# resero-labs/latok

Hardware: AMD Instinct MI355X
Metric: input UTF-8 GB/s tokenized (fused feature+split-mask path) (higher is better)
Workload: dtype u64

## Files before the change

### latok_amd/csrc/api.cpp

```cpp
#include <hip/hip_runtime.h>
#include <errno.h>
#include <fcntl.h>
#include <stdarg.h>
#include <stdio.h>
#include <stdlib.h>
#include <string.h>
#include <sys/mman.h>
#include <sys/stat.h>
#include <unistd.h>

#include <algorithm>
#include <array>
#include <atomic>
#include <chrono>
#include <mutex>
#include <new>
#include <string>
#include <thread>
#include <vector>

#include "../../include/latok_hip.h"
#include "corpus_gen.h"
#include "flow_hazards.h"
#include "kernels.h"
// ... 90 lines not shown
}
static bool wait_completion_word(const unsigned long long* word, unsigned long long seq) {
    const auto t0 = std::chrono::steady_clock::now();
    for (;;) {
        for (int i = 0; i < 256; ++i) {
            if (__atomic_load_n(word, __ATOMIC_ACQUIRE) == seq) return true;
            cpu_relax();
        }
        if (std::chrono::duration_cast<std::chrono::nanoseconds>(std::chrono::steady_clock::now() - t0).count() > kPollNs) return false;
    }
}

static inline size_t align16(size_t x) { return (x + 15) & ~(size_t)15; }

constexpr int64_t kSmallChars = 262144;
constexpr int64_t kSmallStrings = 16384;

enum class Form { Utf32, Latin1, Ucs2, Utf8 };
struct Input {
    const void* p = nullptr;
    Form form = Form::Utf32;
    size_t width() const { return form == Form::Utf32 ? 4 : form == Form::Ucs2 ? 2 : 1; }
    bool narrow() const { return form == Form::Latin1 || form == Form::Ucs2; }
};
static Form form_of_kind(int kind) { return kind == 4 ? Form::Utf32 : kind == 2 ? Form::Ucs2 : kind == 1 ? Form::Latin1 : Form::Utf8; }
struct Batch {
    Input in;
    const int64_t* row = nullptr;
    int64_t n_str = 0, total = 0;
};

struct Workspace {
    DevBuf summ, seg_agg, fix_count, tile_first;
    DevBuf bits, space, kept, wcnt, wpref, bases, scalar, chain, chain_ctl;
    DevBuf codes, widened;
    DevBuf lead, bspace, cpbits, cpspace, cprow;
    DevBuf jbody, jhead;
    unsigned scan_epoch = 0, chain_seen = 0, chain_ctl_seen = 0;
    bool chain_ready = false;
    void release() {
        for (DevBuf* b : {&summ, &seg_agg, &fix_count, &tile_first, &bits, &space, &kept, &wcnt, &wpref, &bases, &scalar, &chain,
                          &chain_ctl, &codes, &widened, &lead, &bspace, &cpbits, &cpspace, &cprow, &jbody, &jhead})
            b->release();
        scan_epoch = chain_seen = chain_ctl_seen = 0;
        chain_ready = false;
    }
};
struct WsNeed {
    DevBuf* buf;
    size_t bytes;
};
constexpr int kTileNeeds = 4;
constexpr int kWsNeeds = 22;
static std::array<WsNeed, kWsNeeds> ws_needs(Workspace& w, int64_t units, bool spans, bool feats, bool widen, int64_t cp_rows = 0,
                                             bool join = false) {
    const size_t t = (size_t)std::max<int64_t>((units + latok::kTile - 1) / latok::kTile, 1);
    const size_t words = (size_t)((units + 63) / 64), c_tiles = (words + 63) / 64;
    return {{{&w.summ, t * 16},
             {&w.seg_agg, (t / latok::kWPB + 2) * (sizeof(latok::Fn64) + sizeof(latok::Hd64))},
             {&w.fix_count, 8},
             {&w.tile_first, t * 8 + 8},
             {&w.bits, words * 8 + 8},
             {&w.space, spans ? words * 8 + 8 : 0},
             {&w.kept, spans ? words * 8 + 8 : 0},
             {&w.wcnt, c_tiles * 8 + 8},
             {&w.wpref, words * 2 + 8},
             {&w.bases, c_tiles * 8 + 8},
             {&w.scalar, 64},
             {&w.chain, (size_t)latok::count_blocks((int64_t)words) * 8 + 64},
             {&w.chain_ctl, 64},
             {&w.codes, feats ? (size_t)units + latok::kTile + 256 : 0},
             {&w.widened, widen ? (size_t)units * 4 + 16 : 0},
             {&w.lead, cp_rows > 0 ? words * 8 + 8 : 0},
             {&w.bspace, cp_rows > 0 && spans ? words * 8 + 8 : 0},
             {&w.cpbits, cp_rows > 0 ? words * 8 + 8 : 0},
             {&w.cpspace, cp_rows > 0 && spans ? words * 8 + 8 : 0},
             {&w.cprow, cp_rows > 0 ? (size_t)cp_rows * 8 : 0},
             {&w.jbody, join ? words * 8 + 8 : 0},
             {&w.jhead, join ? words * 8 + 8 : 0}}};
}
static int ws_ensure(const WsNeed* needs, int n) {
    for (int i = 0; i < n; ++i) {
        const int rc = needs[i].buf->ensure(needs[i].bytes);
        if (rc) return rc;
    }
    return LATOK_OK;
}

struct Ctx {
    std::mutex mu;
    bool inited = false;
    int device = -1, n_cu = 0;
    hipStream_t stream = nullptr;
    DevBuf t1, t1rule, t2code, t2cls, cw;
// ... 106 lines not shown
    hipEvent_t tiles_begin = nullptr, tiles_end = nullptr;
    hipStream_t st = nullptr;
};

int run_pipeline(Ctx& g, Workspace& w, const Pipe& a) {
    const int64_t n_str = a.b.n_str, total = a.b.total;
    if (total <= 0 || n_str <= 0) return LATOK_OK;
    const Input& in = a.b.in;
    int mode = a.mode;
    if (in.form != Form::Utf32) {
        if (mode != latok::kModeBits) return fail(LATOK_ERR_INVALID, "byte-space input supports the bitmask outputs only");
        if (((uintptr_t)in.p & 15) != 0)
            return fail(LATOK_ERR_INVALID, in.narrow() ? "device code-unit pointer must be 16-byte aligned" : "device UTF-8 pointer must be 16-byte aligned");
        mode = in.form == Form::Latin1 ? latok::kModeLatin1 : (in.form == Form::Ucs2 ? latok::kModeUcs2 : latok::kModeBytes);
    }
    if (g.rules_on && mode != latok::kModeBlockMask) mode = latok::mode_with_rules(mode);
    const int64_t n_tiles = (total + latok::kTile - 1) / latok::kTile;
    int rc = ws_ensure(ws_needs(w, total, false, false, false).data(), kTileNeeds);
    if (rc) return rc;
    latok::SplitParams P;
    P.cps = in.form == Form::Utf32 ? (const uint32_t*)in.p : nullptr;
    P.u8 = in.form == Form::Utf32 ? nullptr : (const uint8_t*)in.p;
    P.row_off = a.b.row;
    P.n_str = n_str;
    P.total = total;
    P.n_tiles = n_tiles;
    const int n_cu = g.plan_cus > 0 ? g.plan_cus : g.n_cu;
    const bool one_launch_ok = a.stages == 7 && in.form == Form::Utf32 && !a.tiles_begin && !a.tiles_end && one_segment_enabled();
    latok::LaunchPlan L;
    latok::plan_launch(n_tiles, n_cu, &w != &g.ws, mode, one_launch_ok, &L);
    P.seg_tiles = L.seg_tiles;
    P.n_segs = L.n_segs;
    const bool one_launch = L.one_launch != 0;
    if ((size_t)P.n_segs * (sizeof(latok::Fn64) + sizeof(latok::Hd64)) > w.seg_agg.cap || (size_t)n_tiles * 16 > w.summ.cap)
        return fail(LATOK_ERR_INVALID, "internal: workspace too small for %lld segments / %lld tiles", (long long)P.n_segs, (long long)n_tiles);
    if (a.codes && mode != latok::kModeBits && mode != latok::kModeRules)
        return fail(LATOK_ERR_INVALID, "internal: code bytes are written by the UTF-32 bitmask modes only");
    const uint8_t* tables = (const uint8_t*)((latok::mode_rules(mode) || a.codes) ? g.t1rule.p : g.t1.p);
    P.t1 = tables;
    P.t2 = tables + latok::kStage1Pad;
    if (latok::mode_base(mode) == latok::kModeBytes) {
        P.t1 = (const uint8_t*)(latok::mode_rules(mode) ? g.tb6rule.p : g.tb6.p);
        P.t2 = P.t1 + latok::kB6Stage1Bytes;
    }
    if (latok::mode_rules(mode)) P.rules = g.rules;
    else memset(&P.rules, 0, sizeof(P.rules));
    P.bits_out = a.bits;
    P.values_out = a.values;
    P.space_out = a.space;
    P.lead_out = a.lead;
    P.lead_pref_out = a.lead_pref;
    P.lead_cnt_out = a.lead_cnt;
    P.codes_out = a.codes;
    P.tile_first = (int64_t*)w.tile_first.p;
    P.summ = (int4*)w.summ.p;
    P.seg_fn = (latok::Fn64*)w.seg_agg.p;
    P.seg_hd = (latok::Hd64*)((char*)w.seg_agg.p + (size_t)P.n_segs * sizeof(latok::Fn64));
    P.fix_count = (int64_t*)w.fix_count.p;
    P.bm_a1 = a.bm_a1;
    P.bm_a2 = a.bm_a2;
    P.bm_flags = a.bm_flags;
    P.done = (a.stages & 4) ? a.done : latok::DoneSignal{nullptr, 0, nullptr};
    g.last.plan = L;
    g.last.n_tiles = n_tiles;
    g.last.mode = mode;
    g.last.small = g.pin.d && in.p == g.pin.d;
    g.last.fix_count = (const int64_t*)w.fix_count.p;
    g.last.st = a.st;
    g.last.valid = true;
    const hipStream_t st = a.st;
    if (one_launch) {
        HIP_TRY(latok::launch_one_segment(P, mode, st));
        return LATOK_OK;
    }
    if (a.stages & 1) HIP_TRY(latok::launch_tile_index(P, st));
    if (a.tiles_begin) HIP_TRY(hipEventRecord(a.tiles_begin, st));
    if (a.stages & 2) HIP_TRY(latok::launch_split_tiles(P, mode, L, st));
    if (a.tiles_end) HIP_TRY(hipEventRecord(a.tiles_end, st));
    if (a.stages & 4) HIP_TRY(latok::launch_resolve_fix(P, mode, L, st));
    return LATOK_OK;
}

int check_csr_host(const int64_t* row_off, int64_t n_str, int64_t* total_io) {
    if (n_str < 0) return fail(LATOK_ERR_INVALID, "n_str must be >= 0");
    if (n_str == 0) { *total_io = 0; return LATOK_OK; }
    if (!row_off) return fail(LATOK_ERR_INVALID, "row_off is NULL");
    if (row_off[0] != 0) return fail(LATOK_ERR_INVALID, "row_off[0] must be 0");
    for (int64_t s = 0; s < n_str; ++s)
        if (row_off[s + 1] < row_off[s]) return fail(LATOK_ERR_INVALID, "row_off must be non-decreasing");
    if (*total_io >= 0 && *total_io != row_off[n_str])
        return fail(LATOK_ERR_INVALID, "total_chars does not match row_off[n_str]");
    *total_io = row_off[n_str];
    return LATOK_OK;
}

int resolve_total_device(const int64_t* d_row, int64_t n_str, int64_t* total_io, hipStream_t st) {
    if (n_str < 0) return fail(LATOK_ERR_INVALID, "n_str must be >= 0");
    if (n_str == 0) { *total_io = 0; return LATOK_OK; }
    if (*total_io < 0) {
        HIP_TRY(hipMemcpyAsync(total_io, d_row + n_str, 8, hipMemcpyDeviceToHost, st));
        HIP_TRY(hipStreamSynchronize(st));
    }
    return LATOK_OK;
}

int resolve_total(const int64_t* row_off, int64_t n_str, int64_t* total_io, bool dev, hipStream_t st) {
    return dev ? resolve_total_device(row_off, n_str, total_io, st) : check_csr_host(row_off, n_str, total_io);
}

int arm_done(Ctx& g, hipStream_t st, latok::DoneSignal* done) {
    *done = latok::DoneSignal{nullptr, 0, nullptr};
    if (!poll_completion()) return LATOK_OK;
// ... 1815 lines not shown

int latok_debug_set_scan_epoch(unsigned epoch) {
    LATOK_ENTER();
    g.ws.scan_epoch = epoch & 0x3FFFFu;
    return LATOK_OK;
}

extern "C" int latok_debug_limits(int64_t* out, int n) {
    const int64_t v[15] = {latok::kTile, latok::kWPB, latok::kNarrowWPB, latok::kSegMax, latok::kOneSegTiles, latok::kFastTailTiles,
                           kSmallChars, kSmallStrings, latok::kCompressWaves, latok::kFeatWaves, latok::kFeatRound, latok::kFeatRoundTm,
                           latok::kFeatFormThresh, latok::kFeatWinBytes, latok::kHashWaveBytes};
    if (!out || n < 0) return fail(LATOK_ERR_INVALID, "NULL output");
    const int k = n < 15 ? n : 15;
    for (int i = 0; i < k; ++i) out[i] = v[i];
    return k;
}

static int put_plan(const latok::LaunchPlan& L, int64_t n_tiles, int64_t* out, int n) {
    const int64_t v[12] = {L.n_cu_eff, L.seg_tiles, L.n_segs, L.rounds, L.grid, L.one_launch ? 0 : L.grid, L.fast_tail, L.pf, L.wpb, L.nw,
                           L.one_launch, n_tiles};
    const int k = n < 12 ? n : 12;
    for (int i = 0; i < k; ++i) out[i] = v[i];
    return k;
}

extern "C" int latok_debug_plan(int64_t n_tiles, int n_cu, int in_flow, int mode, int64_t* out, int n) {
    if (!out || n < 0 || n_tiles < 1 || n_cu < 1 || mode < latok::kModeBits || mode > latok::kModeValuesRules)
        return fail(LATOK_ERR_INVALID, "n_tiles >= 1, n_cu >= 1, mode 0..%d", latok::kModeValuesRules);
    latok::LaunchPlan L;
    latok::plan_launch(n_tiles, n_cu, in_flow != 0, mode, one_segment_enabled(), &L);
    return put_plan(L, n_tiles, out, n);
}

extern "C" int latok_debug_set_plan_cus(int n_cu) {
    LATOK_ENTER();
    int rc = need_init(g);
    if (rc) return rc;
    if (n_cu != 0 && (n_cu < 8 || n_cu > g.n_cu)) return fail(LATOK_ERR_INVALID, "plan CUs must be 0 or 8..%d", g.n_cu);
    g.plan_cus = n_cu;
    return LATOK_OK;
}

extern "C" int latok_debug_last_plan(int64_t* out, int n) {
    LATOK_ENTER();
    int rc = need_init(g);
    if (rc) return rc;
    if (!out || n < 0) return fail(LATOK_ERR_INVALID, "NULL output");
    if (!g.last.valid) return 0;
    int64_t fix = 0;
    HIP_TRY(hipStreamSynchronize(g.last.st));
    HIP_TRY(hipMemcpy(&fix, g.last.fix_count, 8, hipMemcpyDeviceToHost));
    const int64_t head[3] = {g.last.mode, g.last.small ? 1 : 0, fix};
    int k = 0;
    for (; k < 3 && k < n; ++k) out[k] = head[k];
    if (n > 3) k += put_plan(g.last.plan, g.last.n_tiles, out + 3, n - 3);
    return k;
}

extern "C" int latok_debug_last_route(void) {
    LATOK_ENTER();
    return g.last_route;
}

extern "C" int latok_debug_flow_route(int n_slots, const uint64_t* lo, const uint64_t* bytes, const int* is_write, int n, int* drained_out) {
    static thread_local latok::FlowHazards held;
    static thread_local unsigned long long seq = 0;
// ... 939 lines not shown
```

### latok_amd/csrc/kernels.h

```cpp
#ifndef LATOK_KERNELS_H
#define LATOK_KERNELS_H
#include <hip/hip_runtime.h>
#include <stdint.h>

#include "split_code.h"

namespace latok {

constexpr int kTile = 4096;
constexpr int kTblShift = 7;
constexpr int kStage1Len = 8705;
constexpr int kStage1Pad = 8720;
constexpr int kStage2Len = 255 * 128;
constexpr int kTablesLdsBytes = kStage1Pad + kStage2Len;
constexpr int kB6Stage1Len = LK_B6_STAGE1_LEN;
constexpr int kB6Stage1Bytes = (kB6Stage1Len * 2 + 1023) / 1024 * 1024;
constexpr int kB6MaxBlocks = 400;
constexpr int kB6Stage2Bytes = kB6MaxBlocks * 64;
constexpr int kB6TablesBytes = kB6Stage1Bytes + kB6Stage2Bytes;
static_assert(kB6Stage1Bytes % 1024 == 0 && kB6Stage2Bytes % 1024 == 0 && kB6Stage1Bytes <= kTablesLdsBytes, "byte space keeps its stage 1 where the other modes keep both stages");
constexpr int kStageBytes = 64 * 80;
constexpr int kWaveLdsBytes = kStageBytes + 16 + 65 * 8 + 8;

constexpr int kModeBits = 0;
// ... 88 lines not shown
};
#if defined(__HIPCC__)
__device__ __forceinline__ int64_t device_total(const int64_t* p, int64_t bound) {
    const int64_t t = *p;
    return t < 0 ? 0 : (t > bound ? bound : t);
}
#endif

struct FeatParams {
    const uint8_t* codes;
    const int64_t* row_off;
    int64_t n_str, total, n_tiles;
    const uint64_t* bits;
    const uint64_t* kept;
    const int64_t* tile_rank;
    const int64_t* tile_cnt;
    const uint16_t* word_pref;
    const int64_t* tile_first;
    const uint64_t* space;
    int8_t* features;
    void* spans4;
    bool out32;
    const int64_t* n_tokens_dev;
    int64_t cap;
    DoneSignal done;
    DeviceTotal dt;
};
hipError_t launch_features_tiles(const FeatParams& P, int n_cu, hipStream_t st);

void plan_segments(int64_t n_tiles, int n_cu, int* seg_tiles, int64_t* n_segs);
constexpr int64_t kOneSegTiles = 24;
constexpr int64_t kFastTailTiles = 256;
constexpr int kNarrowWPB = 16;
constexpr int kCpsPrefetchRows = 2;
constexpr int kCpsPrefetchRowsFlow = 6;
struct LaunchPlan {
    int n_cu_eff;
    int seg_tiles;
    int64_t n_segs;
    int64_t rounds;
    int grid;
    int fast_tail;
    int pf;
    int wpb;
    int nw;
    int one_launch;
};
void plan_launch(int64_t n_tiles, int n_cu, bool in_flow, int mode, bool one_launch_ok, LaunchPlan* L);
hipError_t launch_tile_index(const SplitParams& P, hipStream_t st);
hipError_t launch_split_tiles(const SplitParams& P, int mode, const LaunchPlan& L, hipStream_t st);
hipError_t launch_resolve_fix(const SplitParams& P, int mode, const LaunchPlan& L, hipStream_t st);
hipError_t launch_one_segment(const SplitParams& P, int mode, hipStream_t st);
hipError_t launch_small_batch(const SplitParams& P, bool rules, int kind, bool out32, void* counts, void* items, int8_t* features,
                              int64_t* n_items, unsigned long long* done, unsigned long long seq, hipStream_t st);
hipError_t launch_any_nonzero(const int8_t* a1, const int8_t* a2, int64_t n, int* flags, hipStream_t st);

hipError_t launch_parse_matrix(const uint32_t* cps, int64_t n, const uint8_t* t1, const uint8_t* t2cls,
                               const uint16_t* cw, int8_t* out, hipStream_t st);
constexpr int kSmallMatrixChars = 4096;
hipError_t launch_parse_matrix_small(const uint32_t* cps, int n, const uint8_t* t1, const uint8_t* t2cls, const uint16_t* cw,
                                     int8_t* out, unsigned long long* done, unsigned long long seq, hipStream_t st);
hipError_t launch_combine_rows(const uint8_t* m, int64_t stride_r, int64_t stride_c, int64_t cols, const int8_t* idx,
                               int idx_ndim, int irows, int icols, int8_t* out, hipStream_t st,
                               unsigned long long* done = nullptr, unsigned long long seq = 0);
hipError_t launch_small_block_mask(const SplitParams& P, unsigned long long* done, unsigned long long seq, hipStream_t st);
hipError_t launch_rebase_rows(int64_t* row, int64_t n, int64_t base, hipStream_t st);
int64_t scan_blocks(int64_t n);
hipError_t launch_exclusive_scan(const int64_t* in, int64_t n, int64_t* out, int64_t* total, int64_t* block_tot,
                                 hipStream_t st, int64_t* total_host = nullptr);
int64_t count_blocks(int64_t n_words);
hipError_t launch_word_counts_scan(bool spans, const uint64_t* bits, const uint64_t* space, int64_t n_words, int64_t total,
                                   uint64_t* kept, int64_t* tile_cnt, uint16_t* word_pref, int64_t* tile_rank,
                                   unsigned long long* chain, unsigned* ticket, unsigned epoch, int64_t* total_dev,
                                   int64_t* total_host, int* err, hipStream_t st, DeviceTotal dt = DeviceTotal{nullptr, nullptr});
hipError_t launch_string_counts(bool out32, const uint64_t* mask, const int64_t* tile_rank, const uint16_t* word_pref,
                                const int64_t* row_off, int64_t n_str, int64_t total, const int64_t* n_items, void* counts, int* err,
                                hipStream_t st, DeviceTotal dt = DeviceTotal{nullptr, nullptr});
hipError_t launch_counts_scatter(int kind, bool out32, const uint64_t* bits, const uint64_t* space, const uint64_t* item_mask,
                                 const int64_t* tile_rank, const int64_t* tile_cnt, const uint16_t* word_pref, int64_t n_words,
                                 int64_t total, const int64_t* row_off, int64_t n_str, const int64_t* tile_first, void* out,
                                 const int64_t* n_items_dev, int64_t cap, void* counts, int* err, hipStream_t st, DoneSignal done = DoneSignal{nullptr, 0, nullptr},
                                 DeviceTotal dt = DeviceTotal{nullptr, nullptr});
constexpr int kFeatWaves = 7;
constexpr int kFeatRound = 896;
constexpr int kFeatRec = 25;
// ... 39 lines not shown
```

### latok_amd/csrc/split_kernels.hip

```cpp
#include <hip/hip_runtime.h>
#include <stdint.h>
#include <stdlib.h>

#include "bitscan.h"
#include "kernels.h"
#include "lane_math.h"
#include "utf8_decode.h"

namespace latok {

#ifdef LATOK_STAMPS
__device__ unsigned long long g_stamp_sum[16];
__device__ unsigned long long g_stamp_cnt;
#define LATOK_STAMP(k)                                                                           \
    do {                                                                                         \
        __builtin_amdgcn_sched_barrier(0);                                                       \
        unsigned long long t_;                                                                   \
        asm volatile("s_memtime %0\n\ts_waitcnt lgkmcnt(0)" : "=s"(t_)::"memory");            \
        __builtin_amdgcn_sched_barrier(0);                                                       \
        if ((k) > 0) stamp_acc[(k)] += t_ - stamp_prev;                                          \
        stamp_prev = t_;                                                                         \
    } while (0)
#else
#define LATOK_STAMP(k) do { } while (0)
// ... 1244 lines not shown
        if (tid == 0) { P.seg_fn[seg] = tfn; P.seg_hd[seg] = th; }
    }
    __syncthreads();
}

template <int MODE, bool FAST_TAIL = false, int PF = kCpsPrefetchRows>
__global__ __launch_bounds__(tile_wpb(MODE) * 64) void k_tiles_main(SplitParams P) {
    constexpr int WPB = tile_wpb(MODE);
    __shared__ __attribute__((aligned(16))) uint8_t lds[lds_total_tiles(MODE)];
    const int tid = threadIdx.x;
    const int lane = tid & 63;
    const int wave = __builtin_amdgcn_readfirstlane(tid >> 6);
    if (blockIdx.x == 0 && tid == 0) *P.fix_count = 0;

    bool tables = MODE != kModeBlockMask;
    if (tables) {
        if (mode_base(MODE) == kModeBytes) load_tables_ascii_bytes(lds, P);
        else load_tables<WPB * 64, MODE>(lds, P);
    }
#ifdef LATOK_STAMPS
    unsigned long long stamp_acc[16];
    for (int i = 0; i < 16; ++i) stamp_acc[i] = 0;
#endif
    for (int64_t seg = blockIdx.x; seg < P.n_segs; seg += gridDim.x) {
        run_segment<MODE, FAST_TAIL, WPB, PF>(P, lds, seg, tid, lane, wave, tables LATOK_STAMP_ARG);
        tables = false;
    }
#ifdef LATOK_STAMPS
    if (lane == 0)
        for (int i = 0; i < 16; ++i) atomicAdd(&g_stamp_sum[i], stamp_acc[i]);
#endif
}

template <int MODE, int NW, bool ONE>
__device__ __forceinline__ void resolve_segments(const SplitParams& P, uint8_t* lds, int tid, int lane, int wave) {
    const int S = P.seg_tiles;
    ScanLdsT<NW>& scan = *reinterpret_cast<ScanLdsT<NW>*>(lds + lds_shift(MODE) + kLdsScan);
    int* misc = reinterpret_cast<int*>(lds + lds_shift(MODE) + kLdsMisc);
    int* fix_t = reinterpret_cast<int*>(lds + lds_shift(MODE) + kLdsTf);
    int2* fix_in = reinterpret_cast<int2*>(lds + lds_shift(MODE) + kLdsSumm);
    bool tables_loaded = ONE;

    for (int64_t seg = ONE ? 0 : (int64_t)blockIdx.x; seg < (ONE ? 1 : P.n_segs); seg += ONE ? 1 : (int64_t)gridDim.x) {
        const int64_t T0 = seg * S;
        const int64_t T1 = min(T0 + S, P.n_tiles);
        const int n_seg = (int)(T1 - T0);
        if (tid == 0) misc[0] = 0;
        const int64_t t = T0 + tid;
        int4 s = make_int4(0, 0, 0, 0);
        if (tid < n_seg) s = P.summ[t];
        Fn64 pf = fn_identity();
        Hd64 sh = hd_identity();
        if (P.n_segs > 1) {
            const int64_t per = (P.n_segs + NW * 64 - 1) / (NW * 64);
            const int64_t lo = min((int64_t)tid * per, P.n_segs), hi = min(lo + per, P.n_segs);
            Fn64 f = fn_identity();
            Hd64 h = hd_identity();
            for (int64_t j = lo; j < hi; ++j) {
                if (j < seg) f = fn_then(f, P.seg_fn[j]);
                if (j > seg) h = hd_then(h, P.seg_hd[j]);
            }
            Fn64 ef; Hd64 eh;
            block_scan<NW>(f, h, scan, &ef, &eh, &pf, &sh);
        }
        const long long q_seg_in = fn_apply(pf, 0);
        Hd64 rest; rest.h = sh.h; rest.c = 1;

        Fn64 f = fn_identity();
        Hd64 h = hd_identity();
        if (tid < n_seg) {
            f = fn_of(s);
            h.h = s.z; h.c = s.w & 1;
        }
        Fn64 ef, tfn; Hd64 eh, th;
        block_scan<NW>(f, h, scan, &ef, &eh, &tfn, &th);
        if (tid < n_seg) {
            const long long q_in = fn_apply(ef, q_seg_in);
            const long long q_end = fn_apply(f, q_in);
            const long long h_next = hd_then(eh, rest).h;
            const int tz = (q_end + h_next) > 0;
            const int tz0 = s.y > 0;
            if (q_in != 0 || tz != tz0) {
                const int geom = s.w;
                if (!mode_rules(MODE) && (MODE == kModeBits || mode_is_bytes(MODE)) && (geom & 1) && q_in <= 1 &&
                    (q_in == 0 || s.z == 0)) {
                    const int64_t t0 = t * kTile;
                    const int64_t t_end = min(t0 + kTile, P.total);
                    auto lead_back = [&](int64_t lo, int64_t hi) -> int {
                        int back = 0;
                        if (mode_base(MODE) == kModeBytes && ((geom >> 30) & 1)) {
                            if (hi > t_end) hi = t_end;
                            while (back < 3 && hi - 1 - back > lo && (P.u8[hi - 1 - back] & 0xC0u) == 0x80u) ++back;
                        }
                        return back;
                    };
                    if (q_in == 1) {
                        const int64_t hi = t0 + ((geom >> 1) & 0x1FFF);
                        const int keep = (geom >> 27) & 1;
                        clear_range(P.bits_out, t0, hi, t_end, 0, keep, keep ? lead_back(t0, hi) : 0);
                    }
                    if (tz != tz0) {
                        const int64_t lo = t0 + ((geom >> 14) & 0x1FFF);
                        const int keep = (geom >> 29) & 1;
                        clear_range(P.bits_out, lo, t_end, t_end, (geom >> 28) & 1, keep, keep ? lead_back(lo, t_end) : 0);
                    }
                } else {
                    const int slot = atomicAdd(&misc[0], 1);
                    fix_t[slot] = tid;
                    fix_in[slot] = make_int2((int)(q_in < (1 << 20) ? q_in : (1 << 20)), tz);
                }
            }
        }
        __syncthreads();
        const int n_fix = misc[0];
        if (n_fix > 0) {
            if (!tables_loaded && MODE != kModeBlockMask) {
                load_tables<NW * 64, MODE>(lds, P);
                tables_loaded = true;
                __syncthreads();
            }
            const TileLds L = wave_lds<MODE>(lds, wave);
            for (int i = wave; i < n_fix; i += NW) {
                const int64_t tt = T0 + fix_t[i];
                const int2 in = fix_in[i];
                const int64_t idx0 = wave_lower_bound(P.row_off, P.n_str + 1, tt * kTile, lane);
                process_tile<MODE>(P, L, tt, idx0, in.x, in.y, false, nullptr, lane);
            }
            if (tid == 0) atomicAdd(reinterpret_cast<unsigned long long*>(P.fix_count), (unsigned long long)n_fix);
        }
        __syncthreads();
    }
}

template <int MODE, int NW>
__global__ __launch_bounds__(NW * 64) void k_resolve_fix(SplitParams P) {
    __shared__ __attribute__((aligned(16))) uint8_t lds[lds_total(MODE)];
    const int tid = threadIdx.x;
    const int lane = tid & 63;
    const int wave = __builtin_amdgcn_readfirstlane(tid >> 6);
    resolve_segments<MODE, NW, false>(P, lds, tid, lane, wave);
    signal_block_done(P.done);
}

__device__ __forceinline__ void tile_index_entry(const int64_t* __restrict__ row_off, int64_t n_str, int64_t n_tiles,
                                                 int64_t* __restrict__ tile_first, int64_t s, int lane) {
    int64_t w0 = 0, w1 = -1;
    if (s <= n_str) {
        const int64_t p = row_off[s];
        const int64_t prev = s > 0 ? row_off[s - 1] : -1;
        w0 = prev < 0 ? 0 : prev / kTile + 1;
        w1 = p / kTile;
        if (w1 > n_tiles - 1) w1 = n_tiles - 1;
    }
    const bool wide = w1 - w0 >= 16;
    if (!wide)
        for (int64_t w = w0; w <= w1; ++w) tile_first[w] = s;
    unsigned long long m = __ballot(wide);
    while (m) {
        const int src = __ffsll((long long)m) - 1;
        m &= m - 1;
        const int64_t a = lane_read64(w0, src), b = lane_read64(w1, src), v = lane_read64(s, src);
        for (int64_t w = a + lane; w <= b; w += 64) tile_first[w] = v;
    }
}


template <int MODE>
__global__ __launch_bounds__(kWPB * 64) void k_one_segment(SplitParams P) {
    __shared__ __attribute__((aligned(16))) uint8_t lds[lds_total(MODE)];
    const int tid = threadIdx.x;
    const int lane = tid & 63;
    const int wave = __builtin_amdgcn_readfirstlane(tid >> 6);
    if (tid == 0) *P.fix_count = 0;
    load_tables<kWPB * 64, MODE>(lds, P);
    for (int64_t base = 0; base <= P.n_str; base += kWPB * 64)
        tile_index_entry(P.row_off, P.n_str, P.n_tiles, P.tile_first, base + tid, lane);
    __threadfence_block();
    __syncthreads();
    run_segment<MODE, true>(P, lds, 0, tid, lane, wave, true LATOK_STAMP_NULL);
    __threadfence_block();
    __syncthreads();
    resolve_segments<MODE, kWPB, true>(P, lds, tid, lane, wave);
    signal_block_done(P.done);
}

__global__ void k_any_nonzero(const int8_t* __restrict__ a1, const int8_t* __restrict__ a2, int64_t n,
                              int* __restrict__ flags) {
    int f1 = 0, f2 = 0;
    for (int64_t i = (int64_t)blockIdx.x * blockDim.x + threadIdx.x; i < n; i += (int64_t)gridDim.x * blockDim.x) {
        f1 |= a1[i] != 0;
        f2 |= a2[i] != 0;
    }
    if (__any(f1) && (threadIdx.x & 63) == 0) atomicOr(&flags[0], 1);
    if (__any(f2) && (threadIdx.x & 63) == 0) atomicOr(&flags[1], 1);
}

// ... 732 lines not shown
            f2 |= *reinterpret_cast<const uint32_t*>(P.bm_a2 + i);
        } else {
            for (int64_t j = i; j < n; ++j) { f1 |= (uint8_t)P.bm_a1[j]; f2 |= (uint8_t)P.bm_a2[j]; }
        }
    }
    const int any1 = __any(f1 != 0u), any2 = __any(f2 != 0u);
    if (lane == 0) { s_flags[0] = any1; s_flags[1] = any2; }
    wave_lds_sync();
    P.bm_flags = s_flags;
    process_tile<kModeBlockMask, false, true, true>(P, L, 0, 0, 0, -1, false, nullptr, lane);
    if (S.done) {
        __threadfence_system();
        if (lane == 0) __hip_atomic_store(S.done, S.seq, __ATOMIC_RELAXED, __HIP_MEMORY_SCOPE_SYSTEM);
    }
}

hipError_t launch_small_block_mask(const SplitParams& P, unsigned long long* done, unsigned long long seq, hipStream_t st) {
    SmallParams S;
    S.P = P;
    S.counts = S.items = nullptr;
    S.features = nullptr;
    S.n_items = nullptr;
    S.done = done;
    S.seq = seq;
    hipLaunchKernelGGL(k_small_block_mask, dim3(1), dim3(64), 0, st, S);
    return hipGetLastError();
}

__global__ __launch_bounds__(256) void k_tile_index(const int64_t* __restrict__ row_off, int64_t n_str, int64_t n_tiles,
                                                   int64_t* __restrict__ tile_first) {
    tile_index_entry(row_off, n_str, n_tiles, tile_first, (int64_t)blockIdx.x * blockDim.x + threadIdx.x, threadIdx.x & 63);
}

hipError_t launch_tile_index(const SplitParams& P, hipStream_t st) {
    if (P.n_tiles <= 0) return hipSuccess;
    const int64_t entries = P.n_str + 1;
    hipLaunchKernelGGL(k_tile_index, dim3((unsigned)((entries + 255) / 256)), dim3(256), 0, st, P.row_off, P.n_str, P.n_tiles,
                       P.tile_first);
    return hipGetLastError();
}

void plan_segments(int64_t n_tiles, int n_cu, int* seg_tiles, int64_t* n_segs) {
    const int64_t per_cu = (n_tiles + n_cu - 1) / n_cu;
    const int64_t rounds = per_cu > kSegMax ? (per_cu + kSegMax - 1) / kSegMax : 1;
    int64_t s = (n_tiles + (int64_t)n_cu * rounds - 1) / ((int64_t)n_cu * rounds);
    if (s < kWPB) s = kWPB;
    if (s > kSegMax) s = kSegMax;
    *seg_tiles = (int)s;
    *n_segs = (n_tiles + s - 1) / s;
}

void plan_launch(int64_t n_tiles, int n_cu, bool in_flow, int mode, bool one_launch_ok, LaunchPlan* L) {
    const int wpb = tile_wpb(mode);
    int n_cu_eff = n_cu;
    if (in_flow && n_cu >= 64) {
        const int cand[3] = {n_cu * 7 / 8, n_cu * 13 / 16, n_cu * 3 / 4};
        int best = cand[0], best_fill = -1;
        for (int c = 0; c < 3; ++c) {
            int st_ = 0;
            int64_t ns_ = 0;
            plan_segments(n_tiles, cand[c], &st_, &ns_);
            const int fill = (st_ - 1) % wpb + 1;
            if (fill * 2 >= wpb) { best = cand[c]; break; }
            if (fill > best_fill) { best = cand[c]; best_fill = fill; }
        }
        n_cu_eff = best;
    }
    if (n_cu_eff < 8) n_cu_eff = n_cu < 8 ? n_cu : 8;
    L->n_cu_eff = n_cu_eff;
    plan_segments(n_tiles, n_cu_eff, &L->seg_tiles, &L->n_segs);
    L->one_launch = one_launch_ok && n_tiles <= kOneSegTiles && (mode == kModeBits || mode == kModeRules);
    if (L->one_launch) {
        L->seg_tiles = (int)(n_tiles < kOneSegTiles ? kOneSegTiles : n_tiles);
        L->n_segs = 1;
    }
    L->grid = L->one_launch ? 1 : (int)(L->n_segs < n_cu ? (L->n_segs < 1 ? 1 : L->n_segs) : n_cu);
    L->rounds = (L->n_segs + L->grid - 1) / L->grid;
    L->fast_tail = !L->one_launch && n_tiles <= kFastTailTiles && (mode == kModeBits || mode == kModeRules);
    L->pf = mode == kModeBits && in_flow && !L->fast_tail && !L->one_launch ? kCpsPrefetchRowsFlow : kCpsPrefetchRows;
    L->wpb = L->one_launch ? kWPB : wpb;
    const bool narrow_resolve = mode == kModeBits || mode == kModeBytes || mode == kModeLatin1 || mode == kModeUcs2;
    L->nw = L->one_launch || !narrow_resolve ? kWPB : (L->seg_tiles <= 128 ? 2 : (L->seg_tiles <= 256 ? 4 : kWPB));
}

hipError_t launch_split_tiles(const SplitParams& P, int mode, const LaunchPlan& L, hipStream_t st) {
    const dim3 grid(L.grid), block(kWPB * 64);
    if (mode == kModeBits && L.pf == kCpsPrefetchRowsFlow) hipLaunchKernelGGL((k_tiles_main<kModeBits, false, kCpsPrefetchRowsFlow>), grid, block, 0, st, P);
    else if (mode == kModeBits && L.fast_tail) hipLaunchKernelGGL((k_tiles_main<kModeBits, true>), grid, block, 0, st, P);
    else if (mode == kModeRules && L.fast_tail) hipLaunchKernelGGL((k_tiles_main<kModeRules, true>), grid, block, 0, st, P);
    else if (mode == kModeBits) hipLaunchKernelGGL((k_tiles_main<kModeBits>), grid, block, 0, st, P);
    else if (mode == kModeValues) hipLaunchKernelGGL((k_tiles_main<kModeValues>), grid, block, 0, st, P);
    else if (mode == kModeRules) hipLaunchKernelGGL((k_tiles_main<kModeRules>), grid, block, 0, st, P);
    else if (mode == kModeBytes) hipLaunchKernelGGL((k_tiles_main<kModeBytes>), grid, dim3(tile_wpb(kModeBytes) * 64), 0, st, P);
    else if (mode == kModeLatin1) hipLaunchKernelGGL((k_tiles_main<kModeLatin1>), grid, dim3(tile_wpb(kModeLatin1) * 64), 0, st, P);
    else if (mode == kModeUcs2) hipLaunchKernelGGL((k_tiles_main<kModeUcs2>), grid, dim3(tile_wpb(kModeUcs2) * 64), 0, st, P);
    else if (mode == kModeBytesRules) hipLaunchKernelGGL((k_tiles_main<kModeBytesRules>), grid, block, 0, st, P);
    else if (mode == kModeLatin1Rules) hipLaunchKernelGGL((k_tiles_main<kModeLatin1Rules>), grid, block, 0, st, P);
    else if (mode == kModeUcs2Rules) hipLaunchKernelGGL((k_tiles_main<kModeUcs2Rules>), grid, block, 0, st, P);
    else if (mode == kModeValuesRules) hipLaunchKernelGGL((k_tiles_main<kModeValuesRules>), grid, block, 0, st, P);
    else hipLaunchKernelGGL((k_tiles_main<kModeBlockMask>), grid, block, 0, st, P);
    return hipGetLastError();
}

hipError_t launch_one_segment(const SplitParams& P, int mode, hipStream_t st) {
    if (P.n_segs != 1 || P.seg_tiles < P.n_tiles || P.n_tiles > kOneSegTiles || (mode != kModeBits && mode != kModeRules))
        return hipErrorInvalidValue;
    if (mode == kModeBits) hipLaunchKernelGGL((k_one_segment<kModeBits>), dim3(1), dim3(kWPB * 64), 0, st, P);
    else hipLaunchKernelGGL((k_one_segment<kModeRules>), dim3(1), dim3(kWPB * 64), 0, st, P);
    return hipGetLastError();
}

hipError_t launch_resolve_fix(const SplitParams& P, int mode, const LaunchPlan& L, hipStream_t st) {
    if (L.nw * 64 < P.seg_tiles) return hipErrorInvalidValue;
    const dim3 grid(L.grid), block(kWPB * 64);
#define LATOK_RESOLVE_NW(M)                                                                            \
    if (L.nw == 2) hipLaunchKernelGGL((k_resolve_fix<M, 2>), grid, dim3(128), 0, st, P);               \
    else if (L.nw == 4) hipLaunchKernelGGL((k_resolve_fix<M, 4>), grid, dim3(256), 0, st, P);          \
    else hipLaunchKernelGGL((k_resolve_fix<M, kWPB>), grid, block, 0, st, P)
    if (mode == kModeBits) { LATOK_RESOLVE_NW(kModeBits); }
    else if (mode == kModeValues) hipLaunchKernelGGL((k_resolve_fix<kModeValues, kWPB>), grid, block, 0, st, P);
    else if (mode == kModeRules) hipLaunchKernelGGL((k_resolve_fix<kModeRules, kWPB>), grid, block, 0, st, P);
    else if (mode == kModeBytesRules) hipLaunchKernelGGL((k_resolve_fix<kModeBytesRules, kWPB>), grid, block, 0, st, P);
    else if (mode == kModeLatin1Rules) hipLaunchKernelGGL((k_resolve_fix<kModeLatin1Rules, kWPB>), grid, block, 0, st, P);
    else if (mode == kModeUcs2Rules) hipLaunchKernelGGL((k_resolve_fix<kModeUcs2Rules, kWPB>), grid, block, 0, st, P);
    else if (mode == kModeValuesRules) hipLaunchKernelGGL((k_resolve_fix<kModeValuesRules, kWPB>), grid, block, 0, st, P);
    else if (mode == kModeBytes) { LATOK_RESOLVE_NW(kModeBytes); }
    else if (mode == kModeLatin1) { LATOK_RESOLVE_NW(kModeLatin1); }
    else if (mode == kModeUcs2) { LATOK_RESOLVE_NW(kModeUcs2); }
    else hipLaunchKernelGGL((k_resolve_fix<kModeBlockMask, kWPB>), grid, block, 0, st, P);
#undef LATOK_RESOLVE_NW
    return hipGetLastError();
}

#ifdef LATOK_STAMPS
extern "C" int latok_diag_stamps(unsigned long long* out16, int reset) {
    hipError_t e = hipMemcpyFromSymbol(out16, HIP_SYMBOL(g_stamp_sum), 16 * sizeof(unsigned long long));
    if (reset) {
        unsigned long long z[16] = {0};
        (void)hipMemcpyToSymbol(HIP_SYMBOL(g_stamp_sum), z, sizeof(z));
    }
    return (int)e;
}
#endif

}
```

Before: 1545.

## Split small flow-mode resolve into slim scan plus fix-list recompute on free CUs

For small flow-mode batches, the plan now reserves spare CUs. The resolve stage splits into a slim LDS-light scan kernel that appends tiles needing recomputation to a global fix list, followed by a recompute kernel sized to the free CUs. A wide, unrolled tile-index kernel with shuffled neighbour offsets is also used when free CUs exist. The intent is to shrink LDS and occupancy cost in the resolve pass and balance fix work. The cost is an extra launch, a new workspace buffer and an atomic global counter.

Result: slower. 1512 (-2.1%).

```diff
diff --git a/latok_amd/csrc/api.cpp b/latok_amd/csrc/api.cpp
--- a/latok_amd/csrc/api.cpp
+++ b/latok_amd/csrc/api.cpp
@@ -146,6 +146,7 @@
 
 struct Workspace {
     DevBuf summ, seg_agg, fix_count, tile_first;
+    DevBuf fix_list;
     DevBuf bits, space, kept, wcnt, wpref, bases, scalar, chain, chain_ctl;
     DevBuf codes, widened;
     DevBuf lead, bspace, cpbits, cpspace, cprow;
@@ -153,7 +154,7 @@
     unsigned scan_epoch = 0, chain_seen = 0, chain_ctl_seen = 0;
     bool chain_ready = false;
     void release() {
-        for (DevBuf* b : {&summ, &seg_agg, &fix_count, &tile_first, &bits, &space, &kept, &wcnt, &wpref, &bases, &scalar, &chain,
+        for (DevBuf* b : {&summ, &seg_agg, &fix_count, &tile_first, &fix_list, &bits, &space, &kept, &wcnt, &wpref, &bases, &scalar, &chain,
                           &chain_ctl, &codes, &widened, &lead, &bspace, &cpbits, &cpspace, &cprow, &jbody, &jhead})
             b->release();
         scan_epoch = chain_seen = chain_ctl_seen = 0;
@@ -164,8 +165,8 @@
     DevBuf* buf;
     size_t bytes;
 };
-constexpr int kTileNeeds = 4;
-constexpr int kWsNeeds = 22;
+constexpr int kTileNeeds = 5;
+constexpr int kWsNeeds = 23;
 static std::array<WsNeed, kWsNeeds> ws_needs(Workspace& w, int64_t units, bool spans, bool feats, bool widen, int64_t cp_rows = 0,
                                              bool join = false) {
     const size_t t = (size_t)std::max<int64_t>((units + latok::kTile - 1) / latok::kTile, 1);
@@ -174,6 +175,7 @@
              {&w.seg_agg, (t / latok::kWPB + 2) * (sizeof(latok::Fn64) + sizeof(latok::Hd64))},
              {&w.fix_count, 8},
              {&w.tile_first, t * 8 + 8},
+             {&w.fix_list, t * 16},
              {&w.bits, words * 8 + 8},
              {&w.space, spans ? words * 8 + 8 : 0},
              {&w.kept, spans ? words * 8 + 8 : 0},
@@ -346,7 +348,8 @@
     P.seg_tiles = L.seg_tiles;
     P.n_segs = L.n_segs;
     const bool one_launch = L.one_launch != 0;
-    if ((size_t)P.n_segs * (sizeof(latok::Fn64) + sizeof(latok::Hd64)) > w.seg_agg.cap || (size_t)n_tiles * 16 > w.summ.cap)
+    if ((size_t)P.n_segs * (sizeof(latok::Fn64) + sizeof(latok::Hd64)) > w.seg_agg.cap || (size_t)n_tiles * 16 > w.summ.cap ||
+        (size_t)n_tiles * 16 > w.fix_list.cap)
         return fail(LATOK_ERR_INVALID, "internal: workspace too small for %lld segments / %lld tiles", (long long)P.n_segs, (long long)n_tiles);
     if (a.codes && mode != latok::kModeBits && mode != latok::kModeRules)
         return fail(LATOK_ERR_INVALID, "internal: code bytes are written by the UTF-32 bitmask modes only");
@@ -387,11 +390,11 @@
         HIP_TRY(latok::launch_one_segment(P, mode, st));
         return LATOK_OK;
     }
-    if (a.stages & 1) HIP_TRY(latok::launch_tile_index(P, st));
+    if (a.stages & 1) HIP_TRY(L.free_cus > 0 ? latok::launch_tile_index_wide(P, L.free_cus, st) : latok::launch_tile_index(P, st));
     if (a.tiles_begin) HIP_TRY(hipEventRecord(a.tiles_begin, st));
     if (a.stages & 2) HIP_TRY(latok::launch_split_tiles(P, mode, L, st));
     if (a.tiles_end) HIP_TRY(hipEventRecord(a.tiles_end, st));
-    if (a.stages & 4) HIP_TRY(latok::launch_resolve_fix(P, mode, L, st));
+    if (a.stages & 4) HIP_TRY(L.slim ? latok::launch_resolve_flow(P, mode, L, (int4*)w.fix_list.p, st) : latok::launch_resolve_fix(P, mode, L, st));
     return LATOK_OK;
 }
 
@@ -2273,6 +2276,48 @@
     return put_plan(L, n_tiles, out, n);
 }
 
+static int put_flow_plan(const latok::LaunchPlan& L, int64_t* out, int n) {
+    const int64_t v[5] = {L.free_cus, L.slim, L.one_launch ? 0 : (L.slim ? 2 : 1), L.slim ? L.free_cus : 0, !L.one_launch && L.free_cus > 0};
+    const int k = n < 5 ? n : 5;
+    for (int i = 0; i < k; ++i) out[i] = v[i];
+    return k;
+}
+
+extern "C" int latok_debug_flow_plan(int64_t n_tiles, int n_cu, int in_flow, int mode, int64_t* out, int n) {
+    if (!out || n < 0 || n_tiles < 1 || n_cu < 1 || mode < latok::kModeBits || mode > latok::kModeValuesRules)
+        return fail(LATOK_ERR_INVALID, "n_tiles >= 1, n_cu >= 1, mode 0..%d", latok::kModeValuesRules);
+    latok::LaunchPlan L;
+    latok::plan_launch(n_tiles, n_cu, in_flow != 0, mode, one_segment_enabled(), &L);
+    return put_flow_plan(L, out, n);
+}
+
+extern "C" int latok_debug_last_flow_plan(int64_t* out, int n) {
+    LATOK_ENTER();
+    int rc = need_init(g);
+    if (rc) return rc;
+    if (!out || n < 0) return fail(LATOK_ERR_INVALID, "NULL output");
+    return g.last.valid ? put_flow_plan(g.last.plan, out, n) : 0;
+}
+
+extern "C" int latok_debug_tile_index(const int64_t* row_off_dev, int64_t n_str, int64_t total, int64_t* tile_first_dev, int free_cus) {
+    LATOK_ENTER();
+    int rc = need_init(g);
+    if (rc) return rc;
+    if (!row_off_dev || !tile_first_dev || n_str < 1 || total < 1 || free_cus < 0 || free_cus > g.n_cu)
+        return fail(LATOK_ERR_INVALID, "device buffers, n_str >= 1, total >= 1, free_cus 0..%d", g.n_cu);
+    StreamTurn turn(g, nullptr);
+    latok::SplitParams P;
+    memset(&P, 0, sizeof(P));
+    P.row_off = row_off_dev;
+    P.n_str = n_str;
+    P.total = total;
+    P.n_tiles = (total + latok::kTile - 1) / latok::kTile;
+    P.tile_first = tile_first_dev;
+    HIP_TRY(free_cus > 0 ? latok::launch_tile_index_wide(P, free_cus, turn.st) : latok::launch_tile_index(P, turn.st));
+    HIP_TRY(hipStreamSynchronize(turn.st));
+    return LATOK_OK;
+}
+
 extern "C" int latok_debug_set_plan_cus(int n_cu) {
     LATOK_ENTER();
     int rc = need_init(g);
diff --git a/latok_amd/csrc/kernels.h b/latok_amd/csrc/kernels.h
--- a/latok_amd/csrc/kernels.h
+++ b/latok_amd/csrc/kernels.h
@@ -144,6 +144,7 @@
 constexpr int64_t kOneSegTiles = 24;
 constexpr int64_t kFastTailTiles = 256;
 constexpr int kNarrowWPB = 16;
+constexpr int64_t kFlowSmallTiles = 16384;
 constexpr int kCpsPrefetchRows = 2;
 constexpr int kCpsPrefetchRowsFlow = 6;
 struct LaunchPlan {
@@ -157,12 +158,16 @@
     int wpb;
     int nw;
     int one_launch;
+    int free_cus;
+    int slim;
 };
 void plan_launch(int64_t n_tiles, int n_cu, bool in_flow, int mode, bool one_launch_ok, LaunchPlan* L);
 hipError_t launch_tile_index(const SplitParams& P, hipStream_t st);
 hipError_t launch_split_tiles(const SplitParams& P, int mode, const LaunchPlan& L, hipStream_t st);
 hipError_t launch_resolve_fix(const SplitParams& P, int mode, const LaunchPlan& L, hipStream_t st);
 hipError_t launch_one_segment(const SplitParams& P, int mode, hipStream_t st);
+hipError_t launch_tile_index_wide(const SplitParams& P, int free_cus, hipStream_t st);
+hipError_t launch_resolve_flow(const SplitParams& P, int mode, const LaunchPlan& L, int4* fix_list, hipStream_t st);
 hipError_t launch_small_batch(const SplitParams& P, bool rules, int kind, bool out32, void* counts, void* items, int8_t* features,
                               int64_t* n_items, unsigned long long* done, unsigned long long seq, hipStream_t st);
 hipError_t launch_any_nonzero(const int8_t* a1, const int8_t* a2, int64_t n, int* flags, hipStream_t st);
diff --git a/latok_amd/csrc/split_kernels.hip b/latok_amd/csrc/split_kernels.hip
--- a/latok_amd/csrc/split_kernels.hip
+++ b/latok_amd/csrc/split_kernels.hip
@@ -1300,11 +1300,42 @@
 #endif
 }
 
-template <int MODE, int NW, bool ONE>
-__device__ __forceinline__ void resolve_segments(const SplitParams& P, uint8_t* lds, int tid, int lane, int wave) {
+template <int MODE>
+__device__ __forceinline__ void patch_tile(uint64_t* bits_out, const uint8_t* u8, int64_t total, int64_t t, int geom, bool head, bool tail) {
+    const int64_t t0 = t * kTile;
+    const int64_t t_end = min(t0 + kTile, total);
+    auto lead_back = [&](int64_t lo, int64_t hi) -> int {
+        int back = 0;
+        if (mode_base(MODE) == kModeBytes && ((geom >> 30) & 1)) {
+            if (hi > t_end) hi = t_end;
+            while (back < 3 && hi - 1 - back > lo && (u8[hi - 1 - back] & 0xC0u) == 0x80u) ++back;
+        }
+        return back;
+    };
+    if (head) {
+        const int64_t hi = t0 + ((geom >> 1) & 0x1FFF);
+        const int keep = (geom >> 27) & 1;
+        clear_range(bits_out, t0, hi, t_end, 0, keep, keep ? lead_back(t0, hi) : 0);
+    }
+    if (tail) {
+        const int64_t lo = t0 + ((geom >> 14) & 0x1FFF);
+        const int keep = (geom >> 29) & 1;
+        clear_range(bits_out, lo, t_end, t_end, (geom >> 28) & 1, keep, keep ? lead_back(lo, t_end) : 0);
+    }
+}
+template <int MODE>
+__device__ __attribute__((noinline)) void patch_tile_call(uint64_t* bits_out, const uint8_t* u8, int64_t total, int64_t t, int geom, bool head,
+                                                          bool tail) {
+    patch_tile<MODE>(bits_out, u8, total, t, geom, head, tail);
+}
+
+template <int MODE, int NW, bool ONE, bool LIST = false>
+__device__ __forceinline__ void resolve_segments(const SplitParams& P, uint8_t* lds, int tid, int lane, int wave,
+                                                 int4* __restrict__ fix_list = nullptr) {
     const int S = P.seg_tiles;
-    ScanLdsT<NW>& scan = *reinterpret_cast<ScanLdsT<NW>*>(lds + lds_shift(MODE) + kLdsScan);
-    int* misc = reinterpret_cast<int*>(lds + lds_shift(MODE) + kLdsMisc);
+    uint8_t* const sl = LIST ? lds : lds + lds_shift(MODE) + kLdsScan;
+    ScanLdsT<NW>& scan = *reinterpret_cast<ScanLdsT<NW>*>(sl);
+    int* misc = reinterpret_cast<int*>(sl + (kLdsMisc - kLdsScan));
     int* fix_t = reinterpret_cast<int*>(lds + lds_shift(MODE) + kLdsTf);
     int2* fix_in = reinterpret_cast<int2*>(lds + lds_shift(MODE) + kLdsSumm);
     bool tables_loaded = ONE;
@@ -1342,6 +1373,8 @@
         }
         Fn64 ef, tfn; Hd64 eh, th;
         block_scan<NW>(f, h, scan, &ef, &eh, &tfn, &th);
+        int my_slot = -1;
+        int2 my_in = make_int2(0, 0);
         if (tid < n_seg) {
             const long long q_in = fn_apply(ef, q_seg_in);
             const long long q_end = fn_apply(f, q_in);
@@ -1352,35 +1385,34 @@
                 const int geom = s.w;
                 if (!mode_rules(MODE) && (MODE == kModeBits || mode_is_bytes(MODE)) && (geom & 1) && q_in <= 1 &&
                     (q_in == 0 || s.z == 0)) {
-                    const int64_t t0 = t * kTile;
-                    const int64_t t_end = min(t0 + kTile, P.total);
-                    auto lead_back = [&](int64_t lo, int64_t hi) -> int {
-                        int back = 0;
-                        if (mode_base(MODE) == kModeBytes && ((geom >> 30) & 1)) {
-                            if (hi > t_end) hi = t_end;
-                            while (back < 3 && hi - 1 - back > lo && (P.u8[hi - 1 - back] & 0xC0u) == 0x80u) ++back;
-                        }
-                        return back;
-                    };
-                    if (q_in == 1) {
-                        const int64_t hi = t0 + ((geom >> 1) & 0x1FFF);
-                        const int keep = (geom >> 27) & 1;
-                        clear_range(P.bits_out, t0, hi, t_end, 0, keep, keep ? lead_back(t0, hi) : 0);
-                    }
-                    if (tz != tz0) {
-                        const int64_t lo = t0 + ((geom >> 14) & 0x1FFF);
-                        const int keep = (geom >> 29) & 1;
-                        clear_range(P.bits_out, lo, t_end, t_end, (geom >> 28) & 1, keep, keep ? lead_back(lo, t_end) : 0);
-                    }
+                    if (LIST) patch_tile_call<MODE>(P.bits_out, P.u8, P.total, t, geom, q_in == 1, tz != tz0);
+                    else patch_tile<MODE>(P.bits_out, P.u8, P.total, t, geom, q_in == 1, tz != tz0);
                 } else {
                     const int slot = atomicAdd(&misc[0], 1);
-                    fix_t[slot] = tid;
-                    fix_in[slot] = make_int2((int)(q_in < (1 << 20) ? q_in : (1 << 20)), tz);
+                    const int2 in = make_int2((int)(q_in < (1 << 20) ? q_in : (1 << 20)), tz);
+                    if (LIST) {
+                        my_slot = slot;
+                        my_in = in;
+                    } else {
+                        fix_t[slot] = tid;
+                        fix_in[slot] = in;
+                    }
                 }
             }
         }
         __syncthreads();
         const int n_fix = misc[0];
+        if (LIST) {
+            if (n_fix > 0) {
+                if (tid == 0) misc[1] = (int)atomicAdd(reinterpret_cast<unsigned long long*>(P.fix_count), (unsigned long long)n_fix);
+                __syncthreads();
+                const int64_t at = (int64_t)misc[1] + my_slot;
+                if (my_slot >= 0 && at < P.n_tiles)
+                    fix_list[at] = make_int4((int)(uint32_t)t, (int)(uint32_t)((uint64_t)t >> 32), my_in.x, my_in.y);
+            }
+            __syncthreads();
+            continue;
+        }
         if (n_fix > 0) {
             if (!tables_loaded && MODE != kModeBlockMask) {
                 load_tables<NW * 64, MODE>(lds, P);
@@ -1410,12 +1442,44 @@
     signal_block_done(P.done);
 }
 
-__device__ __forceinline__ void tile_index_entry(const int64_t* __restrict__ row_off, int64_t n_str, int64_t n_tiles,
+template <int MODE, int NW>
+__global__ __launch_bounds__(NW * 64) void k_resolve_slim(SplitParams P, int4* __restrict__ fix_list) {
+    __shared__ __attribute__((aligned(16))) uint8_t lds[kLdsSlice - kLdsScan];
+    const int tid = threadIdx.x;
+    const int lane = tid & 63;
+    const int wave = __builtin_amdgcn_readfirstlane(tid >> 6);
+    resolve_segments<MODE, NW, false, true>(P, lds, tid, lane, wave, fix_list);
+}
+
+template <int MODE>
+__global__ __launch_bounds__(kWPB * 64) void k_resolve_recompute(SplitParams P, const int4* __restrict__ fix_list) {
+    __shared__ __attribute__((aligned(16))) uint8_t lds[lds_total(MODE)];
+    const int tid = threadIdx.x;
+    const int lane = tid & 63;
+    const int wave = __builtin_amdgcn_readfirstlane(tid >> 6);
+    int64_t n_fix = *P.fix_count;
+    if (n_fix > P.n_tiles) n_fix = P.n_tiles;
+    if ((int64_t)blockIdx.x < n_fix) {
+        if (MODE != kModeBlockMask) {
+            load_tables<kWPB * 64, MODE>(lds, P);
+            __syncthreads();
+        }
+        const TileLds L = wave_lds<MODE>(lds, wave);
+        for (int64_t i = (int64_t)wave * gridDim.x + blockIdx.x; i < n_fix; i += (int64_t)kWPB * gridDim.x) {
+            const int4 e = fix_list[i];
+            const int64_t tt = (int64_t)(((uint64_t)(uint32_t)e.y << 32) | (uint32_t)e.x);
+            if (tt < 0 || tt >= P.n_tiles) continue;
+            const int64_t idx0 = wave_lower_bound(P.row_off, P.n_str + 1, tt * kTile, lane);
+            process_tile<MODE>(P, L, tt, idx0, e.z, e.w, false, nullptr, lane);
+        }
+    }
+    signal_block_done(P.done);
+}
+
+__device__ __forceinline__ void tile_index_store(int64_t prev, int64_t p, bool valid, int64_t n_tiles,
                                                  int64_t* __restrict__ tile_first, int64_t s, int lane) {
     int64_t w0 = 0, w1 = -1;
-    if (s <= n_str) {
-        const int64_t p = row_off[s];
-        const int64_t prev = s > 0 ? row_off[s - 1] : -1;
+    if (valid) {
         w0 = prev < 0 ? 0 : prev / kTile + 1;
         w1 = p / kTile;
         if (w1 > n_tiles - 1) w1 = n_tiles - 1;
@@ -1430,6 +1494,15 @@
         const int64_t a = lane_read64(w0, src), b = lane_read64(w1, src), v = lane_read64(s, src);
         for (int64_t w = a + lane; w <= b; w += 64) tile_first[w] = v;
     }
+}
+__device__ __forceinline__ void tile_index_entry(const int64_t* __restrict__ row_off, int64_t n_str, int64_t n_tiles,
+                                                 int64_t* __restrict__ tile_first, int64_t s, int lane) {
+    int64_t p = 0, prev = -1;
+    if (s <= n_str) {
+        p = row_off[s];
+        if (s > 0) prev = row_off[s - 1];
+    }
+    tile_index_store(prev, p, s <= n_str, n_tiles, tile_first, s, lane);
 }
 
 
@@ -2228,6 +2301,43 @@
     tile_index_entry(row_off, n_str, n_tiles, tile_first, (int64_t)blockIdx.x * blockDim.x + threadIdx.x, threadIdx.x & 63);
 }
 
+constexpr int kIndexUnroll = 4;
+__global__ __launch_bounds__(256) void k_tile_index_wide(const int64_t* __restrict__ row_off, int64_t n_str, int64_t n_tiles,
+                                                        int64_t* __restrict__ tile_first) {
+    const int lane = threadIdx.x & 63;
+    constexpr int64_t kChunk = 64 * kIndexUnroll;
+    const int64_t n_chunks = (n_str + kChunk) / kChunk;
+    const int64_t n_waves = (int64_t)gridDim.x * 4;
+    for (int64_t c = (int64_t)blockIdx.x * 4 + (threadIdx.x >> 6); c < n_chunks; c += n_waves) {
+        const int64_t base = c * kChunk;
+        int64_t p[kIndexUnroll];
+#pragma unroll
+        for (int j = 0; j < kIndexUnroll; ++j) {
+            const int64_t s = base + j * 64 + lane;
+            p[j] = s <= n_str ? row_off[s] : 0;
+        }
+        int64_t before = -1;
+        if (lane == 0 && base > 0) before = row_off[base - 1];
+#pragma unroll
+        for (int j = 0; j < kIndexUnroll; ++j) {
+            const int64_t s = base + j * 64 + lane;
+            int64_t prev = (int64_t)__shfl_up((long long)p[j], 1);
+            const int64_t carry = j == 0 ? before : lane_read64(p[j > 0 ? j - 1 : 0], 63);
+            if (lane == 0) prev = carry;
+            tile_index_store(prev, p[j], s <= n_str, n_tiles, tile_first, s, lane);
+        }
+    }
+}
+
+hipError_t launch_tile_index_wide(const SplitParams& P, int free_cus, hipStream_t st) {
+    if (P.n_tiles <= 0) return hipSuccess;
+    const int64_t chunks = (P.n_str + 64 * kIndexUnroll) / (64 * kIndexUnroll);
+    int64_t grid = (chunks + 3) / 4;
+    if (grid > (int64_t)free_cus * 8) grid = (int64_t)free_cus * 8;
+    hipLaunchKernelGGL(k_tile_index_wide, dim3((unsigned)grid), dim3(256), 0, st, P.row_off, P.n_str, P.n_tiles, P.tile_first);
+    return hipGetLastError();
+}
+
 hipError_t launch_tile_index(const SplitParams& P, hipStream_t st) {
     if (P.n_tiles <= 0) return hipSuccess;
     const int64_t entries = P.n_str + 1;
@@ -2277,6 +2387,9 @@
     L->wpb = L->one_launch ? kWPB : wpb;
     const bool narrow_resolve = mode == kModeBits || mode == kModeBytes || mode == kModeLatin1 || mode == kModeUcs2;
     L->nw = L->one_launch || !narrow_resolve ? kWPB : (L->seg_tiles <= 128 ? 2 : (L->seg_tiles <= 256 ? 4 : kWPB));
+    const bool small_flow = in_flow && !L->one_launch && n_tiles <= kFlowSmallTiles;
+    L->free_cus = !small_flow ? 0 : (n_cu > n_cu_eff ? n_cu - n_cu_eff : (n_cu < 8 ? n_cu : 8));
+    L->slim = small_flow && narrow_resolve;
 }
 
 hipError_t launch_split_tiles(const SplitParams& P, int mode, const LaunchPlan& L, hipStream_t st) {
@@ -2328,6 +2441,27 @@
     return hipGetLastError();
 }
 
+hipError_t launch_resolve_flow(const SplitParams& P, int mode, const LaunchPlan& L, int4* fix_list, hipStream_t st) {
+    if (L.nw * 64 < P.seg_tiles || !L.slim || L.free_cus < 1 || !fix_list) return hipErrorInvalidValue;
+    const dim3 grid(L.grid), rgrid(L.free_cus), block(kWPB * 64);
+#define LATOK_RESOLVE_FLOW(M)                                                                                    \
+    {                                                                                                            \
+        if (L.nw == 2) hipLaunchKernelGGL((k_resolve_slim<M, 2>), grid, dim3(128), 0, st, P, fix_list);          \
+        else if (L.nw == 4) hipLaunchKernelGGL((k_resolve_slim<M, 4>), grid, dim3(256), 0, st, P, fix_list);     \
+        else hipLaunchKernelGGL((k_resolve_slim<M, kWPB>), grid, block, 0, st, P, fix_list);                     \
+        hipError_t e = hipGetLastError();                                                                        \
+        if (e != hipSuccess) return e;                                                                           \
+        hipLaunchKernelGGL((k_resolve_recompute<M>), rgrid, block, 0, st, P, (const int4*)fix_list);             \
+    }
+    if (mode == kModeBits) LATOK_RESOLVE_FLOW(kModeBits)
+    else if (mode == kModeBytes) LATOK_RESOLVE_FLOW(kModeBytes)
+    else if (mode == kModeLatin1) LATOK_RESOLVE_FLOW(kModeLatin1)
+    else if (mode == kModeUcs2) LATOK_RESOLVE_FLOW(kModeUcs2)
+    else return hipErrorInvalidValue;
+#undef LATOK_RESOLVE_FLOW
+    return hipGetLastError();
+}
+
 #ifdef LATOK_STAMPS
 extern "C" int latok_diag_stamps(unsigned long long* out16, int reset) {
     hipError_t e = hipMemcpyFromSymbol(out16, HIP_SYMBOL(g_stamp_sum), 16 * sizeof(unsigned long long));
```
